# mountaindust/Parasitoids

Measured on AMD Instinct MI355X. Metric: grid-days/sec on 4096^2 fp64 domain, higher is better.
Workload: dtype f64; 1 GPU; C3 synthetic stack: N=4097 (nominal 4096^2), 30 Gaussian day kernels K=2049, reference torus P=5121, FFT size 5184 (fast mode), prob model, one replica stack per GPU; dom_len=4097, ndays=30, P=5121, fft_len=5184, kernels_direct=False, full_column_pipeline=True

## Files before the change

parasitoids_amd/csrc/fft_kernels.h:

```cpp
#pragma once
#include "fft_core.h"

#define PS_UNROLL 5

struct SrcMap {
  int n1, off1, lo2, off2;
};
__device__ __forceinline__ bool pred_skip(const unsigned long long* pred) {
  return pred && !(__longlong_as_double((long long)*pred) > 1e-8);
}
__device__ __forceinline__ int src_map(const SrcMap& m, int i) {
  if (i < m.n1) return i + m.off1;
  if (i >= m.lo2) return i - m.lo2 + m.off2;
  return -1;
}

struct RowLive {
  int on;
  SrcMap map;
  const int* range;
};
__device__ __forceinline__ bool row_live(const RowLive& v, int r, int batch) {
  if (!v.on) return true;
  const int sr = src_map(v.map, r);
  if (sr < 0) return false;
  if (!v.range) return true;
  return sr >= v.range[2 * batch] && sr <= v.range[2 * batch + 1];
}

struct RowFwdArgs {
  const double* src;
  int64_t src_bstride;
  int src_ld;
  SrcMap rmap, cmap;
  cplx* dst;
  int64_t dst_bstride;
  int H, ld, P;
  int tstride;
  int rp;
  int skip_zero;
  const int* rowrange;
  int nblocks;
  const unsigned long long* pred;
  const unsigned long long* trunc_pred;
  int trunc_n;
  FftProg prog;
};

struct ColArgs {
  const cplx* src;
  const cplx* src2;
  cplx* prod_dst;
  cplx* dst;
  int64_t src_bstride, src2_bstride, prod_bstride, dst_bstride;
  int ld, ncols, wsh, n_outer;
  int in_base_mul, in_stride, out_base_mul, out_stride;
  int tw_mode;
  const cplx* tp_lo;
  const cplx* tp_hi;
  int tp_shift;
  RowLive live;
  int nblocks;
  const unsigned long long* pred;
  FftProg prog;
};

struct RowInvArgs {
  const cplx* src;
  int64_t src_bstride;
  int H, ld, P, N;
  int tstride;
  int pair_src;
  int rp;
  double scale;
  double* rec;
  int64_t rec_bstride;
  double negval, stat_scale;
  double* rowsum;
  long long* rowcnt;
  unsigned long long* padmax;
  double pad_floor;
  int64_t stat_bstride;
  int persistent;
  const int* pad_quiet;
  int nrec;
  double* rec_multi[32];
  FftProg prog;
};

__device__ __forceinline__ int tw_count(const FftProg& P) { return P.n_lo + P.n_hi + P.n_gen; }
__device__ __forceinline__ void load_tw(cplx* tlo, cplx* thi, const FftProg& P) {
  const int n = tw_count(P);
  for (int t = threadIdx.x; t < n; t += blockDim.x) tlo[t] = P.tw_lo[t];
}

template <int DIR, bool GEN, bool BIG>
__device__ __forceinline__ void run_stage_sel(cplx* data, const cplx* tlo, const cplx* thi,
                                              const FftProg& P, int s, int mode, int nb, int wsh,
// ... 881 lines not shown
```

parasitoids_amd/csrc/fft_rs_kernels.h:

```cpp
#pragma once
#include "fft_kernels.h"
#include "fft_rs.h"
#include <type_traits>


template <int R1, int R2, int R3>
struct RsInvLds {
  using S = Rs<R1, R2, R3>;
  static constexpr int XW = (S::XWORDS + 15) & ~15;
  static constexpr int RED = 16 * (S::NTHR / 64);
  static constexpr size_t bytes(int np) { return (size_t)np * (XW + RED) * sizeof(double); }
};

template <int R1, int R2, int R3, int NP>
__global__ void __launch_bounds__((Rs<R1, R2, R3>::NTHR * NP)) k_row_inv_rs(RowInvArgs a) {
  using S = Rs<R1, R2, R3>;
  using Y = RsInvLds<R1, R2, R3>;
  constexpr int L = S::L;
  constexpr int NW = S::NTHR / 64;
  const int half = threadIdx.x / S::NTHR;
  int unit = (int)blockIdx.x;
  if (a.tstride) {
    constexpr int KL = NP >= 4 ? 1 : 4 / NP;
    const int xcd = unit & 7, q = unit >> 3;
// ... 713 lines not shown
        red[wave * 4 + 1] = sb;
        red[wave * 4 + 2] = (double)ca;
        red[wave * 4 + 3] = (double)cb;
        red[4 * NW + wave] = pmax;
      }
      pend = true;
      pend_b = eb;
      pend_ra = era;
    }
    PS_WAIT_VM0();
  };
#undef PS_EPI_PIECE
  auto idle_half = [&]() {
#pragma unroll
    for (int i = 0; i < 9; ++i) PS_BAR_LDS();
  };

  if (role == 0) {
    if (cur < units) {
      prefetch(cur);
      PS_WAIT_VM0();
      loaded = true;
    }
    for (int k = 0; k < n0; ++k) {
      T_half();
      S_half();
    }
    for (int h = 2 * n0; h < HP; ++h) idle_half();
  } else {
    for (int k = 0; k < n1; ++k) {
      S_half();
      T_half();
    }
    int h = 2 * n1;
    if (n1 > 0) {
      S_half();
      ++h;
    }
    for (; h < HP; ++h) idle_half();
  }
  PS_BAR_LDS();
  if (pend && j0 == S::NTHR - 1) finalize();
}


template <int R1, int R2, int R3, int NP>
__global__ void __launch_bounds__((Rs<R1, R2, R3>::NTHR * NP)) k_row_fwd_rs(RowFwdArgs a) {
  using S = Rs<R1, R2, R3>;
  using Y = RsInvLds<R1, R2, R3>;
  constexpr int L = S::L;
  if (pred_skip(a.pred)) return;
  const int half = threadIdx.x / S::NTHR;
  int unit = (int)blockIdx.x;
  if (a.tstride) {
    constexpr int KL = NP >= 4 ? 1 : 4 / NP;
    const int xcd = unit & 7, q = unit >> 3;
    unit = ((q / KL) * 8 + xcd) * KL + (q % KL);
  }
  const int pair = ((int)gridDim.x - 1 - unit) * NP + half;
  const int ra = 2 * pair, rb = ra + 1;
  if (ra >= a.P || pair < 0) return;
  double* ex = reinterpret_cast<double*>(ps_lds_raw) + half * (Y::XW + Y::RED);
  const int j = threadIdx.x - half * S::NTHR;
  const double* src = a.src + (int64_t)blockIdx.y * a.src_bstride;
  cplx* dst = a.dst + (int64_t)blockIdx.y * a.dst_bstride;
  const int rlo = a.rowrange ? a.rowrange[2 * blockIdx.y] : 0;
  const int rhi = a.rowrange ? a.rowrange[2 * blockIdx.y + 1] : 0x7fffffff;
  SrcMap rmap = a.rmap, cmap = a.cmap;
  const bool trunc = a.trunc_pred && !pred_skip(a.trunc_pred);
  if (trunc) {
    rmap.n1 = rmap.n1 < a.trunc_n ? rmap.n1 : a.trunc_n;
    cmap.n1 = cmap.n1 < a.trunc_n ? cmap.n1 : a.trunc_n;
  }
  auto srow = [&](int r) {
    const int sr = r < a.P ? src_map(rmap, r) : -1;
    return (sr < rlo || sr > rhi) ? -1 : sr;
  };
  const int sa = srow(ra), sb = srow(rb);
  const int64_t kst = a.tstride ? (int64_t)a.tstride : 1;
  cplx* da = dst + (a.tstride ? (int64_t)ra : (int64_t)ra * a.ld);
  cplx* db = dst + (a.tstride ? (int64_t)rb : (int64_t)rb * a.ld);
  const bool hasb = rb < a.P;
  if (sa < 0 && sb < 0) {
    const bool cut = trunc && ((ra < a.P && src_map(a.rmap, ra) >= 0) || (rb < a.P && src_map(a.rmap, rb) >= 0));
    if (a.skip_zero && !cut) return;
    const cplx z = make_double2(0.0, 0.0);
    for (int k = j; k < a.H; k += S::NTHR) {
      da[k * kst] = z;
      if (hasb) db[k * kst] = z;
    }
    return;
  }
  const FftProg& P = a.prog;
  const cplx w2 = tw_lookup(P.tw_lo, P.tw_hi, P.tw_shift, S::tw2(j));
  const cplx w3 = tw_lookup(P.tw_lo, P.tw_hi, P.tw_shift, j < S::T3 ? S::tw3(j) : 0);
  cplx x[S::RMAX];
  if (j < S::T1) {
    const double* pa = src + (int64_t)(sa >= 0 ? sa : 0) * a.src_ld;
    const double* pb = src + (int64_t)(sb >= 0 ? sb : 0) * a.src_ld;
#pragma unroll
    for (int q = 0; q < R1; ++q) {
      const int sc = src_map(cmap, j + q * S::T1);
      const bool ok = sc >= 0;
      const int c = ok ? sc : 0;
      const double va = pa[c], vb = pb[c];
      x[q] = make_double2((ok && sa >= 0) ? va : 0.0, (ok && sb >= 0) ? vb : 0.0);
    }
    bfly<R1, PS_FWD>(x);
  }
  rs_tail<S, R1, R2, R3, PS_FWD>(x, ex, j, w2, w3);
  cplx zm[R3 / 2 + 1];
  constexpr int NQ = R3 / 2 + 1;
// ... 33 lines not shown
```

parasitoids_amd/csrc/ps_config.h:

```cpp
#pragma once
#include <cstdlib>
#include <cstring>

#define PS_OPTION_TABLE(X)                                                                          \
                                               \
  X("PS_NO_RS", no_rs, 0, FLAG, C)                                                                  \
  X("PS_NO_RS_FWD", no_rs_fwd, 0, FLAG, C)                                                          \
  X("PS_NO_BIG_RADIX", no_big_radix, 0, FLAG, C)                                                    \
  X("PS_NO_TPIPE", no_tpipe, 0, FLAG, C)                                                            \
  X("PS_NO_FOLD_TPIPE", no_fold_tpipe, 0, FLAG, C)                                                  \
  X("PS_COL_SINGLE_MAX", col_single_max, 1200, INT, C)                                              \
  X("PS_COL_L1", col_l1, 0, INT, C)                                                                 \
  X("PS_CHUNK_DAYS", chunk_days, 0, INT, C)                                                         \
  X("PS_FAST_SIZE", fast_size, 0, INT, C)                                                           \
  X("PS_RS_AREA", rs_area, 0.0, NUM, C)                                                             \
                                                                                 \
  X("PS_COL_WSH", col_wsh, -1, INT, R)                                                              \
  X("PS_COL_THREADS", col_threads, 256, INT, R)                                                     \
  X("PS_FUSED_WSH", fused_wsh, -1, INT, R)                                                          \
  X("PS_FUSED_THREADS", fused_threads, 0, INT, R)                                                   \
  X("PS_FUSED_G", fused_g, 2, INT, R)                                                               \
  X("PS_MULTI_WSH", multi_wsh, -1, INT, R)                                                          \
  X("PS_DUAL_WSH", dual_wsh, -1, INT, R)                                                            \
  X("PS_FUSED_DAYS", fused_days, 8, INT, R)                                                         \
  X("PS_DIRECT_DAYS", direct_days, 4, INT, R)                                                       \
  X("PS_DIRECT_MAX_TERMS", direct_max_terms, 8, INT, R)                                             \
  X("PS_TPIPE_DAYS", tpipe_days, 32, INT, R)                                                        \
  X("PS_DUAL_MIN_DAYS", dual_min_days, 6, INT, R)                                                   \
                                                   \
  X("PS_TINV", tinv, 0, INT, R)                                                                     \
  X("PS_RSP", rsp, -1, INT, R)                                                                      \
  X("PS_ROW2", row2, -1, INT, R)                                                                    \
  X("PS_TPIPE", tpipe, -1, INT, R)                                                                  \
  X("PS_NO_PAIR_ROWS", no_pair_rows, 0, FLAG, R)                                                    \
  X("PS_TPIPE_SPLIT", tpipe_split, 0, INT, R)                                                       \
  X("PS_NO_CONJ", no_conj, 0, FLAG, R)                                                              \
  X("PS_NO_DUAL", no_dual, 0, FLAG, R)                                                              \
  X("PS_NO_DIRECT", no_direct, 0, FLAG, R)                                                          \
  X("PS_NO_ROW_BATCH", no_row_batch, 0, FLAG, R)                                                    \
  X("PS_NO_PAD_QUIET", no_pad_quiet, 0, FLAG, R)                                                    \
  X("PS_NO_TAIL_SPLIT", no_tail_split, 0, FLAG, R)                                                  \
  X("PS_NO_DEFER_REFFT", no_defer_refft, 0, FLAG, R)                                                \
  X("PS_NO_FILTER_CACHE", no_filter_cache, 0, FLAG, R)                                              \
  X("PS_NO_FOLD_FUSE", no_fold_fuse, 0, FLAG, R)                                                    \
  X("PS_NO_FOLD_ALT", no_fold_alt, 0, FLAG, R)                                                      \
  X("PS_NO_FOLD_ROWS", no_fold_rows, 0, FLAG, R)                                                    \
                                                                                 \
  X("PS_NO_SPECULATION", no_speculation, 0, FLAG, R)                                                \
  X("PS_SPEC_DEPTH", spec_depth, 2, INT, R)                                                         \
  X("PS_NO_FLAG_HISTORY", no_flag_history, 0, FLAG, R)                                              \
  X("PS_NO_WINDOW_HINT", no_window_hint, 0, FLAG, R)                                                \
  X("PS_NO_DEFER_CHECK", no_defer_check, 0, FLAG, R)                                                \
  X("PS_FIRST_WINDOW", first_window, -1, INT, R)                                                    \
  X("PS_KT_SPLIT", kt_split, -1, INT, R)                                                            \
  X("PS_NO_LAZY_KT", no_lazy_kt, 0, FLAG, R)                                                        \
  X("PS_NO_WIDE", no_wide, 0, FLAG, R)                                                              \
  X("PS_NO_ROUTE_HISTORY", no_route_history, 0, FLAG, R)                                            \
  X("PS_WIDE_MIN_N", wide_min_n, 1500, INT, R)                                                      \
  X("PS_AUTO_WINDOW", auto_window, 4, INT, R)                                                       \
                                                                  \
  X("PS_PM_SEG", pm_seg, 8, INT, R)                                                                 \
  X("PS_PM_SYNC", pm_sync, 0, FLAG, R)                                                              \
  X("PS_PM_NO_UNROLL", pm_no_unroll, 0, FLAG, R)

struct ps_config {
#define PS_CFG_FIELD_FLAG int
#define PS_CFG_FIELD_INT int
#define PS_CFG_FIELD_NUM double
#define X(key, field, dflt, kind, when) PS_CFG_FIELD_##kind field = dflt;
  PS_OPTION_TABLE(X)
#undef X
};

inline void ps_config_from_env(ps_config* c) {
  *c = ps_config();
#define PS_CFG_ENV_FLAG(field) c->field = (e[0] == '\0' || std::strcmp(e, "0") != 0) ? 1 : 0
#define PS_CFG_ENV_INT(field) c->field = std::atoi(e)
#define PS_CFG_ENV_NUM(field) c->field = std::atof(e)
#define X(key, field, dflt, kind, when) \
  if (const char* e = std::getenv(key)) { PS_CFG_ENV_##kind(field); }
  PS_OPTION_TABLE(X)
#undef X
}

inline int ps_config_set(ps_config* c, const char* key, double value, bool live) {
  if (!key) return -1;
#define PS_CFG_SET_FLAG(field) c->field = value != 0.0 ? 1 : 0
#define PS_CFG_SET_INT(field) c->field = (int)value
#define PS_CFG_SET_NUM(field) c->field = value
#define PS_CFG_WHEN_C true
#define PS_CFG_WHEN_R false
#define X(k, field, dflt, kind, when)         \
  if (std::strcmp(key, k) == 0) {             \
    if (live && PS_CFG_WHEN_##when) return -2; \
    PS_CFG_SET_##kind(field);                 \
    return 0;                                 \
  }
  PS_OPTION_TABLE(X)
#undef X
// ... 15 lines not shown
```

parasitoids_amd/csrc/ps_rs_rows.hip:

```cpp
#include "rs_cfg.h"
#include "rs_launch.h"
#include <algorithm>
#include <cstdlib>

bool rs_lookup(int L, int* r2, int* r3) {
#define X(A, B) if (L == 16 * A * B) { *r2 = A; *r3 = B; return true; }
  PS_RS_SIZES(X)
#undef X
  return false;
}

int rs_next_size(int n) {
  int best = 0;
#define X(A, B) if (16 * A * B >= n && (best == 0 || 16 * A * B < best)) best = 16 * A * B;
  PS_RS_SIZES(X)
#undef X
  return best;
}

bool rs_info(int r2, int r3, RsInfo* out) {
#define X(A, B)                                                                       \
  if (r2 == A && r3 == B) {                                                           \
    using C = RsCfg<A, B>;                                                            \
    *out = RsInfo{C::NP, C::S::NTHR, C::LDS, C::LDSC1, C::LDSC, C::CHAIN, RsPLds<16, A, B>::fits};            \
    return true;                                                                      \
  }
  PS_RS_SIZES(X)
#undef X
  return false;
}

int rs_rows_set_attrs() {
#define X(A, B)                                                                                              \
  {                                                                                                          \
    using C = RsCfg<A, B>;                                                                                   \
    constexpr int np = C::NP;                                                                                \
    using Z = RsPLds<16, A, B>;                                                                              \
    if constexpr (Z::fits) {                                                                                 \
      auto kp = k_row_inv_rsp<16, A, B>;                                                                     \
      if (hipFuncSetAttribute((const void*)kp, hipFuncAttributeMaxDynamicSharedMemorySize, (int)Z::bytes) != hipSuccess) return -1; \
    }                                                                                                        \
    using Z2 = Rs2Lds<16, A, B>;                                                                             \
    if constexpr (Z2::ok) {                                                                                  \
      auto k2 = k_row_inv_rs2<16, A, B>;                                                                     \
      if (Z2::bytes > 48 * 1024 &&                                                                           \
          hipFuncSetAttribute((const void*)k2, hipFuncAttributeMaxDynamicSharedMemorySize, (int)Z2::bytes) != hipSuccess) return -1; \
    }                                                                                                        \
    if (C::LDSC1 > 48 * 1024) {                                                                              \
      auto kr = k_row_inv_fold<16, A, B>;                                                                    \
      if (hipFuncSetAttribute((const void*)kr, hipFuncAttributeMaxDynamicSharedMemorySize, (int)C::LDSC1) != hipSuccess) return -1; \
    }                                                                                                        \
    if (C::LDS > 48 * 1024) {                                                                                \
      auto ki = k_row_inv_rs<16, A, B, np>;                                                                  \
      auto kf = k_row_fwd_rs<16, A, B, np>;                                                                  \
      if (hipFuncSetAttribute((const void*)ki, hipFuncAttributeMaxDynamicSharedMemorySize, (int)C::LDS) != hipSuccess) return -1; \
      if (hipFuncSetAttribute((const void*)kf, hipFuncAttributeMaxDynamicSharedMemorySize, (int)C::LDS) != hipSuccess) return -1; \
    }                                                                                                        \
  }
  PS_RS_SIZES(X)
#undef X
  return 0;
}

static int device_cus();
static int grid_x(int npairs, int np, int tstride) {
  int gx = (npairs + np - 1) / np;
  if (tstride) {
    const int m = 8 * (np >= 4 ? 1 : 4 / np);
    gx = (gx + m - 1) / m * m;
  }
  return gx;
}

int rs_launch_row_fwd(int r2, int r3, const RowFwdArgs& a, int npairs, int batch, hipStream_t st) {
#define X(A, B)                                                                                              \
  if (r2 == A && r3 == B) {                                                                                  \
    using C = RsCfg<A, B>;                                                                                   \
    constexpr int np = C::NP;                                                                                \
                                                 \
    constexpr int np2 = (np >= 2 && C::S::L <= 2560) ? np / 2 : np;                                          \
    if constexpr (np2 != np) {                                                                               \
      const int live = a.rmap.n1 + (a.P > a.rmap.lo2 ? a.P - a.rmap.lo2 : 0);                                \
      if ((((live + 1) / 2 + np - 1) / np) * batch < device_cus()) {                                         \
        auto k2 = k_row_fwd_rs<16, A, B, np2>;                                                               \
        using Y2 = RsInvLds<16, A, B>;                                                                       \
        constexpr size_t lds2 = Y2::bytes(np2);                                                              \
        hipLaunchKernelGGL(k2, dim3(grid_x(npairs, np2, a.tstride), batch), dim3(C::S::NTHR * np2), lds2, st, a); \
        return 1;                                                                                            \
      }                                                                                                      \
    }                                                                                                        \
    auto kern = k_row_fwd_rs<16, A, B, np>;                                                                  \
    hipLaunchKernelGGL(kern, dim3(grid_x(npairs, np, a.tstride), batch), dim3(C::S::NTHR * np), C::LDS, st, a); \
    return 1;                                                                                                \
  }
  PS_RS_SIZES(X)
#undef X
  return 0;
}

int rs_launch_row_fold(int r2, int r3, const RowFoldArgs& a, int units, hipStream_t st) {
#define X(A, B)                                                                                              \
  if (r2 == A && r3 == B) {                                                                                  \
    using C = RsCfg<A, B>;                                                                                   \
    auto kern = k_row_inv_fold<16, A, B>;                                                                    \
    hipLaunchKernelGGL(kern, dim3(units), dim3(C::S::NTHR), C::LDSC1, st, a);                                \
    return 1;                                                                                                \
  }
  PS_RS_SIZES(X)
#undef X
  return 0;
}

static int device_cus() {
  static int n = 0;
  if (n == 0) {
    int dev = 0;
    hipDeviceProp_t prop;
    if (hipGetDevice(&dev) != hipSuccess || hipGetDeviceProperties(&prop, dev) != hipSuccess) return 256;
    n = prop.multiProcessorCount > 0 ? prop.multiProcessorCount : 256;
  }
  return n;
}

int rs_launch_row_inv(int r2, int r3, const RowInvArgs& a, int npairs, int batch, hipStream_t st) {
#define X(A, B)                                                                                              \
  if (r2 == A && r3 == B) {                                                                                  \
    using C = RsCfg<A, B>;                                                                                   \
    using Z = RsPLds<16, A, B>;                                                                              \
    using Z2 = Rs2Lds<16, A, B>;                                                                             \
    if constexpr (Z2::ok) {                                                                                  \
      if (a.persistent == 2 && a.tstride == 0) {         \
        const int units = npairs * batch;                                                                    \
        const int wgs = std::min(device_cus(), (units + 1) / 2);                                             \
        auto k2 = k_row_inv_rs2<16, A, B>;                                                                   \
        hipLaunchKernelGGL(k2, dim3(wgs), dim3(2 * C::S::NTHR), Z2::bytes, st, a, npairs, units);            \
        return 1;                                                                                            \
      }                                                                                                      \
    }                                                                                                        \
    if constexpr (Z::fits) {                                                                                 \
      if (a.persistent && a.tstride == 0) {                                                                  \
        const int units = npairs * batch;                                                                    \
                 \
        constexpr int W = C::S::NTHR / 64;                                                                   \
        constexpr int kw = 8 / W < 1 ? 1 : 8 / W, kl = (int)((size_t)160 * 1024 / Z::bytes);                 \
        constexpr int per_cu = kw < kl ? kw : kl;                                                            \
// ... 17 lines not shown
```

parasitoids_amd/csrc/ps_solver.hip:

```cpp
#include <deque>

#include "chain_kernels.h"
#include "fft_kernels.h"
#include "fft_colfull_kernels.h"
#include "rs_launch.h"
#include "ps_common.h"
#include "ps_config.h"

thread_local std::string ps_tls_error;

extern "C" const char* ps_last_error(void) { return ps_tls_error.c_str(); }
extern "C" int ps_version(void) { return 100; }

extern "C" int ps_device_count(void) {
  int n = 0;
  hipError_t e = hipGetDeviceCount(&n);
  if (e != hipSuccess) return ps_fail(PS_ERR_NO_DEVICE, "hipGetDeviceCount: %s", hipGetErrorString(e));
  return n;
}

extern "C" int ps_device_info(int device, char* name, int n, int* cus, int64_t* hbm_bytes) {
  hipDeviceProp_t p;
  PS_HIP(hipGetDeviceProperties(&p, device));
  if (name && n > 0) snprintf(name, n, "%s (%s)", p.name, p.gcnArchName);
// ... 264 lines not shown
  ~ProfScope() {
    if (!on) return;
    (void)hipEventRecord(r.b, s->stream);
    s->prof_pending.push_back(r);
  }
};

static int settle(ps_solver* s);
static int enter(ps_solver* s) {
  PS_HIP(hipSetDevice(s->device));
  return settle(s);
}

static int row_threads(int L, bool big = false) { return L <= 1024 ? 256 : ((L <= 2560 || big) ? 512 : 1024); }
static int row_pairs(const FftProg& P) {
  int rp = 2048 / std::max(1, P.L);
  rp = std::max(1, std::min(8, rp));
  return rp;
}
static int col_wsh(const ps_solver* s, int L) {
  int w = 4096 / std::max(1, L);
  int sh = 2;
  while ((1 << (sh + 1)) <= w && sh < 5) ++sh;
  if (s->cfg.col_wsh >= 0) sh = s->cfg.col_wsh;
  return sh;
}
static int col_threads(const ps_solver* s) { return s->cfg.col_threads; }

static int set_lds_attr() {
  static bool done = false;
  if (done) return PS_OK;
  const void* ks[] = {(const void*)k_row_fwd<false, false>, (const void*)k_row_fwd<true, false>,
                      (const void*)k_row_fwd<false, true>,
                      (const void*)k_row_inv<false, false>, (const void*)k_row_inv<true, false>,
                      (const void*)k_row_inv<false, true>,
                      (const void*)k_col<PS_FWD, false>, (const void*)k_col<PS_FWD, true>,
                      (const void*)k_col<PS_INV, false>, (const void*)k_col<PS_INV, true>,
                      (const void*)k_col_fused<false>, (const void*)k_col_fused<true>,
                      (const void*)k_col_fused_dual<false>, (const void*)k_col_fused_dual<true>,
#define PS_MULTI_K(ND) \
  (const void*)k_col_fused_multi<false, ND, 1>, (const void*)k_col_fused_multi<true, ND, 1>, \
  (const void*)k_col_fused_multi<false, ND, 2>, (const void*)k_col_fused_multi<true, ND, 2>
                      PS_MULTI_K(1), PS_MULTI_K(2), PS_MULTI_K(4), PS_MULTI_K(8)};
#undef PS_MULTI_K
  for (const void* k : ks) PS_HIP(hipFuncSetAttribute(k, hipFuncAttributeMaxDynamicSharedMemorySize, kMaxLds));
  if (rs_rows_set_attrs() != 0 || rs_colfull_set_attrs() != 0 || rs_coldual_set_attrs() != 0) return ps_fail(PS_ERR_HIP, "hipFuncSetAttribute failed for a register-resident kernel");
  done = true;
  return PS_OK;
}

static int launch_row_fwd(ps_solver* s, const double* src, int64_t src_bstride, int src_ld,
                          SrcMap rmap, SrcMap cmap, cplx* dst, int batch,
                          const unsigned long long* pred, int skip_zero = 0, const int* rowrange = nullptr,
                          const unsigned long long* trunc_pred = nullptr, int trunc_n = 0) {
  RowFwdArgs a;
  if (trunc_pred && s->rs_r2 == 0) return ps_fail(PS_ERR_STATE, "row pass: only the register-resident kernels truncate on the fly");
  a.trunc_pred = trunc_pred; a.trunc_n = trunc_n;
  a.src = src; a.src_bstride = src_bstride; a.src_ld = src_ld;
  a.rmap = rmap; a.cmap = cmap;
  a.dst = dst; a.dst_bstride = (int64_t)s->Pf * s->ld;
  a.H = s->H; a.ld = s->ld; a.P = s->Pf;
  a.tstride = s->tpipe ? s->Pf : 0;
  a.prog = s->row_plan.prog;
  a.rp = row_pairs(a.prog);
  a.pred = pred;
  a.skip_zero = skip_zero;
  a.rowrange = rowrange;
  const int npairs = (s->Pf + 1) / 2;
  a.nblocks = (npairs + a.rp - 1) / a.rp;
  dim3 grid(pred ? std::min(a.nblocks, kPredGrid) : a.nblocks, batch);
  const int thr = row_threads(a.prog.L, s->row_big);
  const size_t lds = ((size_t)a.rp * row_pitch(a.prog) + a.prog.n_lo + a.prog.n_hi + a.prog.n_gen) * sizeof(cplx);
  if (lds > (size_t)kMaxLds) return ps_fail(PS_ERR_UNSUPPORTED, "row pass needs %zu B LDS", lds);
  ProfScope prof(s, pred ? PS_PROF_REFFT : PS_PROF_ROW_FWD);
  if (s->rs_r2 != 0 && !s->cfg.no_rs_fwd) {
    if (!rs_launch_row_fwd(s->rs_r2, s->rs_r3, a, npairs, batch, s->stream))
      return ps_fail(PS_ERR_STATE, "no register-resident row kernel for 16 x %d x %d", s->rs_r2, s->rs_r3);
  } else if (s->row_plan.generic)
    hipLaunchKernelGGL((k_row_fwd<true, false>), grid, dim3(thr), lds, s->stream, a);
  else if (s->row_big)
    hipLaunchKernelGGL((k_row_fwd<false, true>), grid, dim3(thr), lds, s->stream, a);
  else
    hipLaunchKernelGGL((k_row_fwd<false, false>), grid, dim3(thr), lds, s->stream, a);
  PS_HIP(hipGetLastError());
  return PS_OK;
}

template <int DIR>
static int launch_col(ps_solver* s, const ColPass& cp, const cplx* src, const cplx* src2,
                      cplx* prod, cplx* dst, int batch, int64_t src2_bstride,
                      const unsigned long long* pred, RowLive live = RowLive{0, {0, 0, 0, 0}, nullptr}) {
  ColArgs a;
  a.src = src; a.src2 = src2; a.prod_dst = prod; a.dst = dst;
  const int64_t bs = (int64_t)s->Pf * s->ld;
  a.src_bstride = bs; a.src2_bstride = src2_bstride; a.prod_bstride = bs; a.dst_bstride = bs;
  a.ld = s->ld; a.ncols = s->H;
  a.prog = cp.plan->prog;
  a.wsh = col_wsh(s, a.prog.L);
  a.n_outer = cp.n_outer;
  a.in_base_mul = cp.in_base_mul; a.in_stride = cp.in_stride;
  a.out_base_mul = cp.out_base_mul; a.out_stride = cp.out_stride;
  a.tw_mode = cp.tw_mode;
  a.tp_lo = s->tp_lo.p; a.tp_hi = s->tp_hi.p; a.tp_shift = s->tp_shift;
  a.pred = pred;
  a.live = live;
  const int W = 1 << a.wsh;
  const int ntiles = (s->H + W - 1) / W;
  dim3 grid((unsigned)(ntiles * cp.n_outer), batch);
  size_t lds = (((size_t)a.prog.L << a.wsh) + a.prog.n_lo + a.prog.n_hi + a.prog.n_gen + a.prog.L) * sizeof(cplx) + (size_t)a.prog.L * sizeof(int);
  while (lds > (size_t)kMaxLds && a.wsh > 0) {
    --a.wsh;
    lds = (((size_t)a.prog.L << a.wsh) + a.prog.n_lo + a.prog.n_hi + a.prog.n_gen + a.prog.L) * sizeof(cplx) + (size_t)a.prog.L * sizeof(int);
  }
  if (lds > (size_t)kMaxLds) return ps_fail(PS_ERR_UNSUPPORTED, "column pass needs %zu B LDS", lds);
  {
    const int W2 = 1 << a.wsh;
    a.nblocks = ((s->H + W2 - 1) / W2) * cp.n_outer;
    grid.x = (unsigned)(pred ? std::min(a.nblocks, kPredGrid) : a.nblocks);
  }
  ProfScope prof(s, pred ? PS_PROF_REFFT
                          : (DIR == PS_FWD ? PS_PROF_COL_FWD_A : PS_PROF_COL_INV_A) + (cp.second ? 1 : 0));
  if (cp.plan->generic)
    hipLaunchKernelGGL((k_col<DIR, true>), grid, dim3(col_threads(s)), lds, s->stream, a);
  else
    hipLaunchKernelGGL((k_col<DIR, false>), grid, dim3(col_threads(s)), lds, s->stream, a);
  PS_HIP(hipGetLastError());
  return PS_OK;
}

// ... 86 lines not shown
      return ps_fail(PS_ERR_STATE, "full-column pass: an alternative state source needs a plain single-day pass");
    a.alt_src = alt->src; a.alt_pred = alt->pred; a.alt_live = alt->live;
  }
  if (s->refft_pending) {
    if (!(mode == 0 && nd == 1 && batch == 1 && !pred && state == s->Ahat.p))
      return ps_fail(PS_ERR_STATE, "full-column pass: a flagged day's re-transform is still pending");
    a.alt_src = s->Trow.p; a.alt_pred = s->refft_pending;
    a.alt_live = RowLive{1, map_plain(s->N, s->Pf), nullptr};
  }
  a.pad_row0 = 2 * ((s->N + 1) / 2);
  a.ncols_total = s->H;
  a.col0 = col0;
  const int64_t spec = (int64_t)s->Pf * s->ld;
  a.src = src; a.src_bstride = spec;
  a.state = state; a.state_bstride = state_bstride >= 0 ? state_bstride : spec;
  a.dst = dst; a.dst_bstride = spec;
  a.ld = s->ld; a.ncols = ncols >= 0 ? ncols : s->H; a.mode = mode; a.store_prod = store_prod;
  a.nd = nd; a.src_dstride = spec; a.dst_dstride = spec;
  colfull_set_layout(a, s->tinv ? 1 : inter_layout(s), s->Pf);
  a.live = live;
  a.pred = pred;
  a.prog = s->row_plan.prog;
  const int groups = (a.ncols - col0 + 7) / 8;
  const int lines8 = (groups + 7) / 8;
  if (mode == 2) a.pad_energy = pad_energy;
  const bool prof_was = s->prof_on;
  if (!timed) s->prof_on = false;
  ProfScope prof(s, pred ? PS_PROF_REFFT
                          : (mode == 1 ? PS_PROF_COL_FWD_A
                                       : (nd == 2 ? PS_PROF_COL_INV_A2 : nd == 4 ? PS_PROF_COL_INV_A4
                                          : nd == 8 ? PS_PROF_COL_INV_A8 : nd == 1 ? PS_PROF_COL_INV_A : PS_PROF_COL_INV_AN)),
                 nd);
  s->prof_on = prof_was;
  if (mode == 0 && !pred && store_prod && colfull_dual(s, nd)) {
    a.pad_energy = pad_energy;
    if (!rs_launch_coldual(s->rs_r2, s->rs_r3, a, lines8, batch, s->stream))
      return ps_fail(PS_ERR_STATE, "two-role full-column pass: size 16 x %d x %d is not served", s->rs_r2, s->rs_r3);
    PS_HIP(hipGetLastError());
    return PS_OK;
  }
  if (!rs_launch_colfull(s->rs_r2, s->rs_r3, a, lines8, batch, s->stream))
    return ps_fail(PS_ERR_UNSUPPORTED, "full-column pass: size 16 x %d x %d cannot run this (chained days need the state column in LDS)",
                   s->rs_r2, s->rs_r3);
  PS_HIP(hipGetLastError());
  return PS_OK;
}

static bool colfull_chains(const ps_solver* s) {
  RsInfo info;
  return rs_info(s->rs_r2, s->rs_r3, &info) && info.chain;
}

static int fwd2d(ps_solver* s, const double* src, int64_t src_bstride, int src_ld, SrcMap rmap,
                 SrcMap cmap, cplx* out, int batch, const unsigned long long* pred, const int* rowrange = nullptr) {
  PS_TRY(launch_row_fwd(s, src, src_bstride, src_ld, rmap, cmap, s->T1.p, batch, pred, 1, rowrange));
  if (s->tpipe) return launch_colfull(s, 1, s->T1.p, out, 0, nullptr, batch, RowLive{1, rmap, rowrange}, pred);
  if (s->fwd_passes.size() == 1) {
    PS_TRY(launch_col<PS_FWD>(s, s->fwd_passes[0], s->T1.p, nullptr, nullptr, out, batch, 0, pred, RowLive{1, rmap, rowrange}));
  } else {
    PS_TRY(launch_col<PS_FWD>(s, s->fwd_passes[0], s->T1.p, nullptr, nullptr, s->T2.p, batch, 0, pred, RowLive{1, rmap, rowrange}));
    PS_TRY(launch_col<PS_FWD>(s, s->fwd_passes[1], s->T2.p, nullptr, nullptr, out, batch, 0, pred));
  }
  return PS_OK;
}

static int inv2d(ps_solver* s, const cplx* A, const cplx* B, cplx* prod, double* rec,
                 int stat_slot, double negval, double stat_scale) {
  if (s->tpipe) {
    if (B || prod) return ps_fail(PS_ERR_STATE, "inv2d: product form is not used by the full-column pipeline");
    PS_TRY(launch_colfull(s, 2, nullptr, const_cast<cplx*>(A), 0, s->T1.p, 1, RowLive{0, {0, 0, 0, 0}, nullptr}, nullptr));
    return launch_row_inv(s, s->T1.p, rec, stat_slot, 1, negval, stat_scale);
  }
  if (s->inv_passes.size() == 1) {
    PS_TRY(launch_col<PS_INV>(s, s->inv_passes[0], A, B, prod, s->T1.p, 1, 0, nullptr));
    PS_TRY(launch_row_inv(s, s->T1.p, rec, stat_slot, 1, negval, stat_scale));
  } else {
    PS_TRY(launch_col<PS_INV>(s, s->inv_passes[0], A, B, prod, s->T1.p, 1, 0, nullptr));
    PS_TRY(launch_col<PS_INV>(s, s->inv_passes[1], s->T1.p, nullptr, nullptr, s->T2.p, 1, 0, nullptr));
    PS_TRY(launch_row_inv(s, s->T2.p, rec, stat_slot, 1, negval, stat_scale));
  }
  return PS_OK;
}

static int fwd2d_partial(ps_solver* s, const double* src, int64_t src_bstride, int src_ld,
                         SrcMap rmap, SrcMap cmap, cplx* out, int batch, const int* rowrange = nullptr,
                         bool direct = false) {
  const RowLive live{1, rmap, rowrange};
  s->kt_live = RowLive{0, {0, 0, 0, 0}, nullptr};
  s->kt_direct = s->split && direct && !s->tpipe;
  if (s->tpipe) {
    s->kt_live = live;
    return launch_row_fwd(s, src, src_bstride, src_ld, rmap, cmap, out, batch, nullptr, 1, rowrange);
  }
  if (!s->split || direct) {
    s->kt_live = live;
    return launch_row_fwd(s, src, src_bstride, src_ld, rmap, cmap, out, batch, nullptr, 1, rowrange);
  }
  PS_TRY(launch_row_fwd(s, src, src_bstride, src_ld, rmap, cmap, s->T1.p, batch, nullptr, 1, rowrange));
  return launch_col<PS_FWD>(s, s->fwd_passes[0], s->T1.p, nullptr, nullptr, out, batch, 0, nullptr, live);
}

static void fused_direct_args(ps_solver* s, ColFusedArgs& a) {
  a.direct = s->kt_direct ? 1 : 0;
  a.no_conj = s->cfg.no_conj;
  a.tp_lo = s->tp_lo.p; a.tp_hi = s->tp_hi.p; a.tp_shift = s->tp_shift;
  a.mgL2 = ps_magic((uint32_t)a.L2);
}
static size_t fused_direct_lds(const ColFusedArgs& a) { return a.direct ? ((size_t)a.L1 + a.L2 + 1) * sizeof(cplx) + 64 : 0; }

static int launch_col_fused(ps_solver* s, const cplx* kt, cplx* state, int store_prod, cplx* dst,
                            const int* rowrange) {
  ColFusedArgs a;
  DevPlan* plan = s->split ? &s->col_plan2 : &s->col_plan1;
  a.src = kt; a.state = state; a.dst = dst;
  a.src_bstride = 0;
  a.ld = s->ld; a.ncols = s->H;
  a.L1 = s->split ? s->L1 : 1;
  a.L2 = s->split ? s->L2 : s->Pf;
  a.store_prod = store_prod;
  a.live = s->kt_live;
  a.live.range = rowrange;
  a.prog = plan->prog;
  a.dst_dstride = 0;
  a.live2 = RowLive{0, {0, 0, 0, 0}, nullptr};
  fused_direct_args(s, a);
  a.wsh = std::min(col_wsh(s, a.prog.L), 4);
  if (s->cfg.fused_wsh >= 0) a.wsh = s->cfg.fused_wsh;
  auto need = [&](int wsh) {
    return (((size_t)a.prog.L << wsh) + a.prog.n_lo + a.prog.n_hi + a.prog.n_gen) * sizeof(cplx) +
           (size_t)(a.prog.L + 4) * sizeof(int) + fused_direct_lds(a);
  };
  while (need(a.wsh) > (size_t)kMaxLds && a.wsh > 0) --a.wsh;
  if (need(a.wsh) > (size_t)kMaxLds) return ps_fail(PS_ERR_UNSUPPORTED, "column pass needs %zu B LDS", need(a.wsh));
  const int W = 1 << a.wsh;
  const int ntiles = (s->H + W - 1) / W;
  dim3 grid((unsigned)((a.direct ? (ntiles + 7) / 8 * 8 : ntiles) * a.L1), 1);
  ProfScope prof(s, PS_PROF_COL_INV_A);
  const int fthr = s->cfg.fused_threads > 0 ? s->cfg.fused_threads : col_threads(s);
  if (plan->generic)
    hipLaunchKernelGGL(k_col_fused<true>, grid, dim3(fthr), need(a.wsh), s->stream, a);
  else
    hipLaunchKernelGGL(k_col_fused<false>, grid, dim3(fthr), need(a.wsh), s->stream, a);
  PS_HIP(hipGetLastError());
  return PS_OK;
}

static int launch_col_fused_multi(ps_solver* s, const cplx* kt, int nd, cplx* state, cplx* dst,
                                  const int* rowrange, int* done) {
  ColFusedArgs a;
  DevPlan* plan = s->split ? &s->col_plan2 : &s->col_plan1;
  const int64_t spec = (int64_t)s->Pf * s->ld;
// ... 534 lines not shown
  if (!st.ev) PS_HIP(hipEventCreateWithFlags(&st.ev, hipEventDisableTiming));
  char* hv = st.p;
  char* hr = hv + (size_t)nnz * 8;
  char* hc = hr + (size_t)nnz * 4;
  std::memcpy(hv, val, (size_t)nnz * 8);
  std::memcpy(hr, row, (size_t)nnz * 4);
  std::memcpy(hc, col, (size_t)nnz * 4);
  PS_HIP(hipMemcpyAsync(s->orow.p, hr, nnz * 4, hipMemcpyHostToDevice, s->stream));
  PS_HIP(hipMemcpyAsync(s->ocol.p, hc, nnz * 4, hipMemcpyHostToDevice, s->stream));
  PS_HIP(hipMemcpyAsync(s->oval.p, hv, nnz * 8, hipMemcpyHostToDevice, s->stream));
  PS_HIP(hipEventRecord(st.ev, s->stream));
  st.busy = true;
  ++s->n_staged_uploads;
  return PS_OK;
}

static int set_state_scatter(ps_solver* s, const int* row, const int* col, const double* val, int64_t nnz, int off,
                             bool known_rows) {
  const bool fresh = s->recs[PS_REC_STATE].empty() || !s->recs[PS_REC_STATE][0];
  PS_TRY(ensure_record(s, PS_REC_STATE, 0));
  PS_TRY(ensure_temps(s, 1));
  double* rec = s->recs[PS_REC_STATE][0];
  if (known_rows && s->srange_valid && !fresh && s->mode != PS_MODE_FOLD) {
    const int lo = std::max(s->hsrange[0], 0), hi = std::min(s->hsrange[1], s->N - 1);
    if (lo <= hi) PS_HIP(hipMemsetAsync(rec + (size_t)lo * s->N, 0, (size_t)(hi - lo + 1) * s->N * sizeof(double), s->stream));
  } else {
    PS_HIP(hipMemsetAsync(rec, 0, (size_t)s->N * s->N * sizeof(double), s->stream));
  }
  s->srange_valid = false;
  PS_TRY(scatter_from_device(s, row, col, val, nnz, rec, s->N, off));
  if (s->mode == PS_MODE_FOLD) {
    PS_TRY(s->torus.ensure((size_t)s->Pref * s->Pref));
    PS_HIP(hipMemsetAsync(s->torus.p, 0, (size_t)s->Pref * s->Pref * sizeof(double), s->stream));
    PS_HIP(hipMemcpy2DAsync(s->torus.p, (size_t)s->Pref * sizeof(double), rec, (size_t)s->N * sizeof(double),
                            (size_t)s->N * sizeof(double), (size_t)s->N, hipMemcpyDeviceToDevice, s->stream));
    s->have_state = true;
    return PS_OK;
  }
  s->spec_valid = false;
  s->have_state = true;
  return PS_OK;
}

int ps_solver_set_state_device_coo(ps_solver* s, const int* row, const int* col, const double* val,
                                   int64_t nnz, int off) {
  return set_state_scatter(s, row, col, val, nnz, off, false);
}

static int ensure_spectrum(ps_solver* s) {
  if (s->spec_valid || s->mode == PS_MODE_FOLD) return PS_OK;
  if (s->recs[PS_REC_STATE].empty() || !s->recs[PS_REC_STATE][0]) return ps_fail(PS_ERR_STATE, "no state record");
  PS_TRY(ensure_temps(s, 1));
  PS_TRY(fwd2d(s, s->recs[PS_REC_STATE][0], 0, s->N, map_plain(s->N, s->Pf), map_plain(s->N, s->Pf), s->Ahat.p, 1, nullptr,
               s->srange_valid ? s->srange.p : nullptr));
  s->spec_valid = true;
  return PS_OK;
}

static void set_pipeline(ps_solver* s, bool tpipe) {
  if (!s->tpipe_ok) tpipe = false;
  if (s->tpipe == tpipe) return;
  s->tpipe = tpipe;
  s->bhat_first = -1;
  s->bhat_count = 0;
  s->filt_keys.clear();
}

extern "C" int ps_solver_set_state_coo(ps_solver* s, const int32_t* row, const int32_t* col,
                                       const double* val, int64_t nnz) {
  if (!s || nnz < 0 || (nnz > 0 && (!row || !col || !val))) return ps_fail(PS_ERR_BAD_ARG, "set_state_coo: bad arguments");
  PS_HIP(hipSetDevice(s->device));
  PS_TRY(check_coo(row, col, nnz, s->N, "state"));
  PS_TRY(upload_coo(s, row, col, val, nnz));
  PS_TRY(set_state_scatter(s, s->orow.p, s->ocol.p, s->oval.p, nnz, 0, true));
  int range[2] = {1, 0};
  for (int64_t i = 0; i < nnz; ++i) {
    if (range[0] > range[1]) range[0] = range[1] = row[i];
    range[0] = std::min(range[0], (int)row[i]);
    range[1] = std::max(range[1], (int)row[i]);
  }
  PS_TRY(s->srange.ensure(2));
  hipLaunchKernelGGL(k_set_int2, dim3(1), dim3(64), 0, s->stream, s->srange.p, range[0], range[1]);
  PS_HIP(hipGetLastError());
  s->hsrange[0] = range[0];
  s->hsrange[1] = range[1];
  s->srange_valid = true;
  return PS_OK;
}

static bool direct_possible(const ps_solver* s) {
  return s->split && s->mode != PS_MODE_FOLD && !s->cfg.no_direct &&
         s->L1 <= 255 && s->L2 <= 255;
}
static bool day_is_compact(const ps_solver* s, int d) {
  const int max_terms = s->cfg.direct_max_terms;
  const int M = s->Kmax / 2;
  const int lo = s->hkrange[2 * d], hi = s->hkrange[2 * d + 1];
  if (lo > hi) return true;
  const int below = std::max(0, std::min(hi, M - 1) - lo + 1), above = std::max(0, hi - std::max(lo, M) + 1);
  const int terms = (below + s->L2 - 1) / s->L2 + (above + s->L2 - 1) / s->L2;
  return terms <= max_terms;
}

static int transform_kernels(ps_solver* s, int first, int count, int slot0, int total, int direct_chunk) {
  const int K = s->Kmax, M = K / 2;
  const size_t spec = (size_t)s->Pf * s->ld;
  if (total < 0) total = count;
  PS_TRY(s->kdense.ensure((size_t)total * K * K));
  PS_TRY(s->Bhat.ensure(spec * total));
  PS_TRY(ensure_temps(s, total));
  double* kd = s->kdense.p + (size_t)slot0 * K * K;
  int maxrows = 0;
  int64_t maxn = 0;
  for (int d = first; d < first + count; ++d) {
    maxrows = std::max(maxrows, std::min(s->hkrange[2 * d + 1], K - 1) - std::max(s->hkrange[2 * d], 0) + 1);
    maxn = std::max<int64_t>(maxn, s->koff[d + 1] - s->koff[d]);
  }
  if (maxrows > 0) {
    const int64_t n = (int64_t)maxrows * K;
    const int blocks = (int)std::min<int64_t>((n + 255) / 256, 2048);
    hipLaunchKernelGGL(k_zero_band, dim3(blocks, count), dim3(256), 0, s->stream, kd, K, s->krange.p + 2 * first);
    PS_HIP(hipGetLastError());
  }
  if (maxn > 0) {
    const int thr = 256;
    const int blocks = (int)std::min<int64_t>((maxn + thr - 1) / thr, 1024);
    hipLaunchKernelGGL(k_scatter_coo_batch, dim3(blocks, count), dim3(thr), 0, s->stream, s->krow.p, s->kcol.p,
                       s->kval.p, s->dkoff.p, s->dkshape.p, first, kd, K);
    PS_HIP(hipGetLastError());
  }
  bool direct = direct_possible(s);
  if (direct_chunk >= 0) direct = direct && direct_chunk != 0;
  else for (int d = first; d < first + count && direct; ++d) direct = day_is_compact(s, d);
  PS_TRY(fwd2d_partial(s, kd, (int64_t)K * K, K, map_wrap(M, s->Pf), map_wrap(M, s->Pf), s->Bhat.p + (size_t)slot0 * spec, count,
                       s->krange.p + 2 * first, direct));
  s->bhat_first = first - slot0;
  s->bhat_count = slot0 + count;
  return PS_OK;
}

static int transform_kernels(ps_solver* s, int first, int count, int slot0 = 0, int total = -1, int direct_chunk = -1);
static int kernels_ready(ps_solver* s, int d) {
  if (s->kt_lazy_from >= 0 && d >= s->kt_lazy_from) {
    const int from = s->kt_lazy_from, done = from - s->kt_lazy_c0;
    s->kt_lazy_from = -1;
    PS_TRY(transform_kernels(s, from, s->kt_lazy_cn - done, done, s->kt_lazy_cn, s->kt_lazy_direct));
  }
  if (s->kt_from >= 0 && d >= s->kt_from) {
    PS_HIP(hipStreamWaitEvent(s->stream, s->kt_ev, 0));
    s->kt_from = -1;
  }
  return PS_OK;
}

static int drain_kernel_readers(ps_solver* s) {
  PS_TRY(enter(s));
  if (s->stream2) PS_HIP(hipStreamSynchronize(s->stream2));
  PS_HIP(hipStreamSynchronize(s->stream));
  return PS_OK;
}

static int set_kernels_common(ps_solver* s, int nk, const int64_t* off, const int32_t* kshape,
                              const int32_t* rows) {
  s->koff.assign(off, off + nk + 1);
  s->kshape.assign(kshape, kshape + nk);
  s->nk = nk;
  s->Kmax = 1;
  for (int d = 0; d < nk; ++d) {
    if (kshape[d] < 1 || kshape[d] % 2 == 0)
      return ps_fail(PS_ERR_BAD_SHAPE, "kernel %d has even/invalid shape %d (CalcSol.py:58)", d, kshape[d]);
    if (kshape[d] / 2 > s->M)
      return ps_fail(PS_ERR_BAD_SHAPE, "kernel %d shape %d exceeds max_shape %d", d, kshape[d], 2 * s->M + 1);
    s->Kmax = std::max(s->Kmax, kshape[d]);
  }
  if (2 * (s->Kmax / 2) + 1 > s->Pf) return ps_fail(PS_ERR_BAD_SHAPE, "kernel larger than the pad");
  s->hkrange.assign(2 * (size_t)std::max(nk, 1), 0);
  const int M = s->Kmax / 2;
  for (int d = 0; d < nk; ++d) {
    const int o = M - kshape[d] / 2;
    int lo = 0, hi = kshape[d] - 1;
    if (rows && off[d + 1] > off[d]) {
      lo = kshape[d];
      hi = -1;
      for (int64_t i = off[d]; i < off[d + 1]; ++i) {
        lo = std::min(lo, (int)rows[i]);
        hi = std::max(hi, (int)rows[i]);
      }
    } else if (rows) {
// ... 1393 lines not shown
```

parasitoids_amd/csrc/rs_launch.h:

```cpp
#pragma once
#include <hip/hip_runtime.h>
#include "fft_kernels.h"

struct ColFullArgs;

struct RsInfo {
  int np, nthr;
  size_t lds_rows, lds_col1, lds_colc;
  bool chain;
  bool rsp;
};
bool rs_lookup(int L, int* r2, int* r3);
int rs_next_size(int n);
bool rs_info(int r2, int r3, RsInfo* out);
int rs_rows_set_attrs();
int rs_colfull_set_attrs();
int rs_launch_row_fwd(int r2, int r3, const RowFwdArgs& a, int npairs, int batch, hipStream_t st);
int rs_launch_row_inv(int r2, int r3, const RowInvArgs& a, int npairs, int batch, hipStream_t st);
int rs_launch_colfull(int r2, int r3, const ColFullArgs& a, int lines8, int batch, hipStream_t st);
struct RowFoldArgs;
int rs_launch_row_fold(int r2, int r3, const RowFoldArgs& a, int units, hipStream_t st);
bool rs_colfull_alt_ok(int r2, int r3);
bool rs_dual_ok(int r2, int r3);
int rs_coldual_set_attrs();
int rs_launch_coldual(int r2, int r3, const ColFullArgs& a, int lines8, int batch, hipStream_t st);
```

Measured before the change: 4352 grid-days/s.

## Size row-forward FFT grid to live source rows using host row ranges

New measurement: 4388 grid-days/s, median of 6. Within noise of the previous version (+0.8%).

```diff
diff --git a/parasitoids_amd/csrc/fft_kernels.h b/parasitoids_amd/csrc/fft_kernels.h
--- a/parasitoids_amd/csrc/fft_kernels.h
+++ b/parasitoids_amd/csrc/fft_kernels.h
@@ -1,11 +1,9 @@
 #pragma once
 #include "fft_core.h"
+#include "live_grid.h"
 
 #define PS_UNROLL 5
 
-struct SrcMap {
-  int n1, off1, lo2, off2;
-};
 __device__ __forceinline__ bool pred_skip(const unsigned long long* pred) {
   return pred && !(__longlong_as_double((long long)*pred) > 1e-8);
 }
@@ -44,6 +42,7 @@
   const unsigned long long* pred;
   const unsigned long long* trunc_pred;
   int trunc_n;
+  int live_grid;
   FftProg prog;
 };
 
diff --git a/parasitoids_amd/csrc/fft_rs_kernels.h b/parasitoids_amd/csrc/fft_rs_kernels.h
--- a/parasitoids_amd/csrc/fft_rs_kernels.h
+++ b/parasitoids_amd/csrc/fft_rs_kernels.h
@@ -789,12 +789,18 @@
   if (pred_skip(a.pred)) return;
   const int half = threadIdx.x / S::NTHR;
   int unit = (int)blockIdx.x;
+  constexpr int KL = NP >= 4 ? 1 : 4 / NP;
   if (a.tstride) {
-    constexpr int KL = NP >= 4 ? 1 : 4 / NP;
-    const int xcd = unit & 7, q = unit >> 3;
-    unit = ((q / KL) * 8 + xcd) * KL + (q % KL);
-  }
-  const int pair = ((int)gridDim.x - 1 - unit) * NP + half;
+    unit = live_grid_xcd_remap(unit, KL);
+  }
+  int aunit = (int)gridDim.x - 1 - unit;
+  if (a.live_grid) {
+    const int kl = a.tstride ? KL : 1;
+    const LiveGrid g = live_grid_of(a.rmap, a.P, a.rowrange[2 * blockIdx.y], a.rowrange[2 * blockIdx.y + 1], NP, kl);
+    aunit = live_grid_unit(g, kl, unit);
+    if (aunit < 0) return;
+  }
+  const int pair = aunit * NP + half;
   const int ra = 2 * pair, rb = ra + 1;
   if (ra >= a.P || pair < 0) return;
   double* ex = reinterpret_cast<double*>(ps_lds_raw) + half * (Y::XW + Y::RED);
diff --git a/parasitoids_amd/csrc/live_grid.h b/parasitoids_amd/csrc/live_grid.h
--- /dev/null
+++ b/parasitoids_amd/csrc/live_grid.h
@@ -0,0 +1,58 @@
+#pragma once
+#include "fft_core.h"
+
+struct SrcMap {
+  int n1, off1, lo2, off2;
+};
+
+struct LiveGrid {
+  int g1hi, n1, g2hi, n2;
+};
+
+PS_HD LiveGrid live_grid_of(const SrcMap& m, int P, int lo, int hi, int np, int kl) {
+  const int R = 2 * np * kl;
+  int a1 = lo - m.off1, b1 = hi - m.off1 + 1;
+  a1 = a1 > 0 ? a1 : 0;
+  b1 = b1 < m.n1 ? b1 : m.n1;
+  b1 = b1 < P ? b1 : P;
+  int a2 = lo - m.off2, b2 = m.lo2 + hi - m.off2 + 1;
+  a2 = m.lo2 + (a2 > 0 ? a2 : 0);
+  b2 = b2 < P ? b2 : P;
+  if (b1 > a1 && a2 < b1) a2 = b1;
+  LiveGrid g{0, 0, 0, 0};
+  int g1lo = 0, g2lo = 0;
+  if (b1 > a1) {
+    g1lo = a1 / R;
+    g.g1hi = (b1 - 1) / R;
+    g.n1 = g.g1hi - g1lo + 1;
+  }
+  if (b2 > a2) {
+    g2lo = a2 / R;
+    g.g2hi = (b2 - 1) / R;
+    if (g.n1 > 0 && g2lo == g.g1hi) ++g2lo;
+    g.n2 = g.g2hi - g2lo + 1;
+  }
+  return g;
+}
+
+PS_HD int live_grid_units(const LiveGrid& g, int kl) { return (g.n1 + g.n2) * kl; }
+
+PS_HD int live_grid_dim(int units, int kl, bool colmajor) {
+  if (!colmajor) return units;
+  const int m = 8 * kl;
+  return (units + m - 1) / m * m;
+}
+
+PS_HD int live_grid_unit(const LiveGrid& g, int kl, int cu) {
+  const int t = cu / kl, w = cu - t * kl;
+  int ag;
+  if (t < g.n2) ag = g.g2hi - t;
+  else if (t < g.n2 + g.n1) ag = g.g1hi - (t - g.n2);
+  else return -1;
+  return ag * kl + (kl - 1 - w);
+}
+
+PS_HD int live_grid_xcd_remap(int block, int kl) {
+  const int xcd = block & 7, q = block >> 3;
+  return ((q / kl) * 8 + xcd) * kl + (q % kl);
+}
diff --git a/parasitoids_amd/csrc/ps_config.h b/parasitoids_amd/csrc/ps_config.h
--- a/parasitoids_amd/csrc/ps_config.h
+++ b/parasitoids_amd/csrc/ps_config.h
@@ -45,6 +45,7 @@
   X("PS_NO_FOLD_FUSE", no_fold_fuse, 0, FLAG, R)                                                    \
   X("PS_NO_FOLD_ALT", no_fold_alt, 0, FLAG, R)                                                      \
   X("PS_NO_FOLD_ROWS", no_fold_rows, 0, FLAG, R)                                                    \
+  X("PS_NO_LIVE_GRID", no_live_grid, 0, FLAG, R)                                                    \
                                                                                  \
   X("PS_NO_SPECULATION", no_speculation, 0, FLAG, R)                                                \
   X("PS_SPEC_DEPTH", spec_depth, 2, INT, R)                                                         \
diff --git a/parasitoids_amd/csrc/ps_rs_rows.hip b/parasitoids_amd/csrc/ps_rs_rows.hip
--- a/parasitoids_amd/csrc/ps_rs_rows.hip
+++ b/parasitoids_amd/csrc/ps_rs_rows.hip
@@ -72,7 +72,15 @@
   return gx;
 }
 
-int rs_launch_row_fwd(int r2, int r3, const RowFwdArgs& a, int npairs, int batch, hipStream_t st) {
+static int live_grid_x(const RowFwdArgs& a, const int* hrange, int batch, int np) {
+  const int kl = a.tstride ? (np >= 4 ? 1 : 4 / np) : 1;
+  int units = 0;
+  for (int b = 0; b < batch; ++b)
+    units = std::max(units, live_grid_units(live_grid_of(a.rmap, a.P, hrange[2 * b], hrange[2 * b + 1], np, kl), kl));
+  return live_grid_dim(units, kl, a.tstride != 0);
+}
+
+int rs_launch_row_fwd(int r2, int r3, const RowFwdArgs& a, int npairs, int batch, const int* hrange, hipStream_t st) {
 #define X(A, B)                                                                                              \
   if (r2 == A && r3 == B) {                                                                                  \
     using C = RsCfg<A, B>;                                                                                   \
@@ -85,12 +93,14 @@
         auto k2 = k_row_fwd_rs<16, A, B, np2>;                                                               \
         using Y2 = RsInvLds<16, A, B>;                                                                       \
         constexpr size_t lds2 = Y2::bytes(np2);                                                              \
-        hipLaunchKernelGGL(k2, dim3(grid_x(npairs, np2, a.tstride), batch), dim3(C::S::NTHR * np2), lds2, st, a); \
+        const int gx = a.live_grid ? live_grid_x(a, hrange, batch, np2) : grid_x(npairs, np2, a.tstride);    \
+        if (gx > 0) hipLaunchKernelGGL(k2, dim3(gx, batch), dim3(C::S::NTHR * np2), lds2, st, a);            \
         return 1;                                                                                            \
       }                                                                                                      \
     }                                                                                                        \
     auto kern = k_row_fwd_rs<16, A, B, np>;                                                                  \
-    hipLaunchKernelGGL(kern, dim3(grid_x(npairs, np, a.tstride), batch), dim3(C::S::NTHR * np), C::LDS, st, a); \
+    const int gx = a.live_grid ? live_grid_x(a, hrange, batch, np) : grid_x(npairs, np, a.tstride);          \
+    if (gx > 0) hipLaunchKernelGGL(kern, dim3(gx, batch), dim3(C::S::NTHR * np), C::LDS, st, a);             \
     return 1;                                                                                                \
   }
   PS_RS_SIZES(X)
diff --git a/parasitoids_amd/csrc/ps_solver.hip b/parasitoids_amd/csrc/ps_solver.hip
--- a/parasitoids_amd/csrc/ps_solver.hip
+++ b/parasitoids_amd/csrc/ps_solver.hip
@@ -340,7 +340,8 @@
 static int launch_row_fwd(ps_solver* s, const double* src, int64_t src_bstride, int src_ld,
                           SrcMap rmap, SrcMap cmap, cplx* dst, int batch,
                           const unsigned long long* pred, int skip_zero = 0, const int* rowrange = nullptr,
-                          const unsigned long long* trunc_pred = nullptr, int trunc_n = 0) {
+                          const unsigned long long* trunc_pred = nullptr, int trunc_n = 0,
+                          const int* hrange = nullptr) {
   RowFwdArgs a;
   if (trunc_pred && s->rs_r2 == 0) return ps_fail(PS_ERR_STATE, "row pass: only the register-resident kernels truncate on the fly");
   a.trunc_pred = trunc_pred; a.trunc_n = trunc_n;
@@ -354,6 +355,7 @@
   a.pred = pred;
   a.skip_zero = skip_zero;
   a.rowrange = rowrange;
+  a.live_grid = (hrange && rowrange && skip_zero && !pred && !trunc_pred && !s->cfg.no_live_grid) ? 1 : 0;
   const int npairs = (s->Pf + 1) / 2;
   a.nblocks = (npairs + a.rp - 1) / a.rp;
   dim3 grid(pred ? std::min(a.nblocks, kPredGrid) : a.nblocks, batch);
@@ -362,7 +364,7 @@
   if (lds > (size_t)kMaxLds) return ps_fail(PS_ERR_UNSUPPORTED, "row pass needs %zu B LDS", lds);
   ProfScope prof(s, pred ? PS_PROF_REFFT : PS_PROF_ROW_FWD);
   if (s->rs_r2 != 0 && !s->cfg.no_rs_fwd) {
-    if (!rs_launch_row_fwd(s->rs_r2, s->rs_r3, a, npairs, batch, s->stream))
+    if (!rs_launch_row_fwd(s->rs_r2, s->rs_r3, a, npairs, batch, hrange, s->stream))
       return ps_fail(PS_ERR_STATE, "no register-resident row kernel for 16 x %d x %d", s->rs_r2, s->rs_r3);
   } else if (s->row_plan.generic)
     hipLaunchKernelGGL((k_row_fwd<true, false>), grid, dim3(thr), lds, s->stream, a);
@@ -555,8 +557,9 @@
 }
 
 static int fwd2d(ps_solver* s, const double* src, int64_t src_bstride, int src_ld, SrcMap rmap,
-                 SrcMap cmap, cplx* out, int batch, const unsigned long long* pred, const int* rowrange = nullptr) {
-  PS_TRY(launch_row_fwd(s, src, src_bstride, src_ld, rmap, cmap, s->T1.p, batch, pred, 1, rowrange));
+                 SrcMap cmap, cplx* out, int batch, const unsigned long long* pred, const int* rowrange = nullptr,
+                 const int* hrange = nullptr) {
+  PS_TRY(launch_row_fwd(s, src, src_bstride, src_ld, rmap, cmap, s->T1.p, batch, pred, 1, rowrange, nullptr, 0, hrange));
   if (s->tpipe) return launch_colfull(s, 1, s->T1.p, out, 0, nullptr, batch, RowLive{1, rmap, rowrange}, pred);
   if (s->fwd_passes.size() == 1) {
     PS_TRY(launch_col<PS_FWD>(s, s->fwd_passes[0], s->T1.p, nullptr, nullptr, out, batch, 0, pred, RowLive{1, rmap, rowrange}));
@@ -587,19 +590,19 @@
 
 static int fwd2d_partial(ps_solver* s, const double* src, int64_t src_bstride, int src_ld,
                          SrcMap rmap, SrcMap cmap, cplx* out, int batch, const int* rowrange = nullptr,
-                         bool direct = false) {
+                         bool direct = false, const int* hrange = nullptr) {
   const RowLive live{1, rmap, rowrange};
   s->kt_live = RowLive{0, {0, 0, 0, 0}, nullptr};
   s->kt_direct = s->split && direct && !s->tpipe;
   if (s->tpipe) {
     s->kt_live = live;
-    return launch_row_fwd(s, src, src_bstride, src_ld, rmap, cmap, out, batch, nullptr, 1, rowrange);
+    return launch_row_fwd(s, src, src_bstride, src_ld, rmap, cmap, out, batch, nullptr, 1, rowrange, nullptr, 0, hrange);
   }
   if (!s->split || direct) {
     s->kt_live = live;
-    return launch_row_fwd(s, src, src_bstride, src_ld, rmap, cmap, out, batch, nullptr, 1, rowrange);
-  }
-  PS_TRY(launch_row_fwd(s, src, src_bstride, src_ld, rmap, cmap, s->T1.p, batch, nullptr, 1, rowrange));
+    return launch_row_fwd(s, src, src_bstride, src_ld, rmap, cmap, out, batch, nullptr, 1, rowrange, nullptr, 0, hrange);
+  }
+  PS_TRY(launch_row_fwd(s, src, src_bstride, src_ld, rmap, cmap, s->T1.p, batch, nullptr, 1, rowrange, nullptr, 0, hrange));
   return launch_col<PS_FWD>(s, s->fwd_passes[0], s->T1.p, nullptr, nullptr, out, batch, 0, nullptr, live);
 }
 
@@ -1240,7 +1243,7 @@
   if (s->recs[PS_REC_STATE].empty() || !s->recs[PS_REC_STATE][0]) return ps_fail(PS_ERR_STATE, "no state record");
   PS_TRY(ensure_temps(s, 1));
   PS_TRY(fwd2d(s, s->recs[PS_REC_STATE][0], 0, s->N, map_plain(s->N, s->Pf), map_plain(s->N, s->Pf), s->Ahat.p, 1, nullptr,
-               s->srange_valid ? s->srange.p : nullptr));
+               s->srange_valid ? s->srange.p : nullptr, s->srange_valid ? s->hsrange : nullptr));
   s->spec_valid = true;
   return PS_OK;
 }
@@ -1321,7 +1324,7 @@
   if (direct_chunk >= 0) direct = direct && direct_chunk != 0;
   else for (int d = first; d < first + count && direct; ++d) direct = day_is_compact(s, d);
   PS_TRY(fwd2d_partial(s, kd, (int64_t)K * K, K, map_wrap(M, s->Pf), map_wrap(M, s->Pf), s->Bhat.p + (size_t)slot0 * spec, count,
-                       s->krange.p + 2 * first, direct));
+                       s->krange.p + 2 * first, direct, s->hkrange.data() + 2 * first));
   s->bhat_first = first - slot0;
   s->bhat_count = slot0 + count;
   return PS_OK;
diff --git a/parasitoids_amd/csrc/rs_launch.h b/parasitoids_amd/csrc/rs_launch.h
--- a/parasitoids_amd/csrc/rs_launch.h
+++ b/parasitoids_amd/csrc/rs_launch.h
@@ -15,7 +15,7 @@
 bool rs_info(int r2, int r3, RsInfo* out);
 int rs_rows_set_attrs();
 int rs_colfull_set_attrs();
-int rs_launch_row_fwd(int r2, int r3, const RowFwdArgs& a, int npairs, int batch, hipStream_t st);
+int rs_launch_row_fwd(int r2, int r3, const RowFwdArgs& a, int npairs, int batch, const int* hrange, hipStream_t st);
 int rs_launch_row_inv(int r2, int r3, const RowInvArgs& a, int npairs, int batch, hipStream_t st);
 int rs_launch_colfull(int r2, int r3, const ColFullArgs& a, int lines8, int batch, hipStream_t st);
 struct RowFoldArgs;
```
